# GRIPS-code/pyLBL

Measured on AMD Instinct MI355X. Metric: line×gridpoint Voigt evals/sec (whole job; per GPU: evals_per_s_per_gpu; spectra/sec: spectra_per_s), higher is better.
Workload: dtype f64; 1 GPU; BASELINE config 'target': 1 level(s) per GPU, H2O+CO2, grid 1-5000 cm-1 at 0.001 cm-1 (5000000 points), cut_off 25, remove_pedestal=False; levels_total=1, atmosphere=surface, output=gas, parallelism=levels sharded

## Files before the change

### pylbl_amd/abi.py

```python
from ctypes import CDLL, POINTER, Structure, byref, c_char_p, c_double, c_int32, c_int64, \
                   c_void_p
import os
from pathlib import Path

import numpy as np

from .errors import EngineError

LIBRARY_PATH = Path(__file__).resolve().parent / "liblbl_amd.so"

LBL_OK = 0
TABLE_OPEN_FAILED, TABLE_NO_ALIAS, TABLE_NO_TIPS, TABLE_NOT_RECTANGULAR, TABLE_NO_ISOTOPOLOGUES, \
    TABLE_NO_TRANSITIONS = 10, 11, 12, 13, 14, 15
RANGE_REFERENCE, RANGE_SKIP = 0, 1
PREP_DEVICE, PREP_HOST = 0, 1
OUT_DEVICE, ASYNC, SCALE_DENSITY, ACCUMULATE, FARFIELD, DEFER_FINISH = 1, 2, 4, 8, 16, 32
RANGE_POLICIES = {"reference": RANGE_REFERENCE, "skip": RANGE_SKIP}
PATH_OPTICAL_DEPTH, PATH_TRANSMITTANCE, PATH_CUMULATIVE, PATH_FROM_LAST, PATH_CONTINUE = \
    0x100, 0x200, 0x400, 0x800, 0x1000
PATH_RADIANCE, PATH_BRIGHTNESS = 0x2000, 0x4000
PATH_FLUX_UP = 0x8000
PATH_JACOBIAN_DEPTH, PATH_JACOBIAN_LOG_DEPTH, PATH_JACOBIAN_TEMPERATURE, \
    PATH_JACOBIAN_BOUNDARY_T, PATH_JACOBIAN_BOUNDARY_E = \
    0x10000, 0x20000, 0x40000, 0x80000, 0x100000
# ... 116 lines not shown
    "lbl_path_thermal_two_stream_source": _BLOCK + [_i32] + _RUN + [_ptr, _ptr, _f64, _ptr, _ptr,
                                                                    _ptr, _i32] + [_ptr]*10 +
                                          [_i32],
}
KDIST_PROTOTYPES = {
    "lbl_band_distribution_weighted": [_ptr, _ptr, _i64, _i64, _i32, _ptr, _i32, _ptr, _i32,
                                       _ptr, _ptr, _ptr, _ptr, _i64, _ptr, _ptr, _ptr, _i32,
                                       _ptr, _ptr, _ptr, _ptr, _ptr, _i32, _ptr, _i32],
}
SCATTERER_PROTOTYPES = {
    "lbl_path_two_stream_spectral": _BLOCK + _RUN + [_ptr, _i32, _i32, _ptr, _ptr] + [_ptr]*5 +
                                    [_i32] + [_ptr]*18 + [_i32],
    "lbl_path_thermal_two_stream_spectral": _BLOCK + [_i32] + _RUN + [_ptr, _ptr, _i32, _ptr, _ptr,
                                                                      _f64, _ptr, _ptr, _ptr,
                                                                      _i32] + [_ptr]*10 + [_i32],
}
THERMAL_RADIANCE_PROTOTYPES = {
    "lbl_path_thermal_radiance": _BLOCK + [_i32] + _RUN + [_ptr, _f64] + [_ptr]*6 + [_i32] +
                                 [_ptr]*4 + [_i32],
}
SOLAR_RADIANCE_PROTOTYPES = {
    "lbl_path_solar_radiance": _BLOCK + _RUN + [_ptr]*11 + [_i32] + [_ptr]*3 + [_i32],
}
SCATTERER_RADIANCE_PROTOTYPES = {
    "lbl_path_thermal_radiance_spectral": _BLOCK + [_i32] + _RUN + [_ptr, _i32, _ptr, _ptr, _f64] +
                                          [_ptr]*6 + [_i32] + [_ptr]*4 + [_i32],
    "lbl_path_solar_radiance_spectral": _BLOCK + _RUN + [_ptr, _i32, _i32, _ptr, _ptr] +
                                        [_ptr]*10 + [_i32] + [_ptr]*3 + [_i32],
}
THERMAL_RADIANCE_SOURCE_PROTOTYPES = {
    "lbl_path_thermal_radiance_source": _BLOCK + [_i32] + _RUN + [_ptr, _ptr, _f64] + [_ptr]*6 +
                                        [_i32] + [_ptr]*4 + [_i32],
}

_library = None


def _preload_hip_runtime():
    import importlib.util
    import os
    import sys
    from ctypes import RTLD_GLOBAL
    if "torch" in sys.modules:
        return
    try:
        spec = importlib.util.find_spec("torch")
    except (ImportError, ValueError):
        spec = None
    if spec is None or not spec.submodule_search_locations:
        return
    for location in spec.submodule_search_locations:
        candidate = os.path.join(location, "lib", "libamdhip64.so")
        if os.path.exists(candidate):
            try:
                CDLL(candidate, mode=RTLD_GLOBAL)
            except OSError:
                pass
            return


def library():
    global _library
    if _library is not None:
        return _library
    path = LIBRARY_PATH
    if os.environ.get("PYLBL_AMD_LIBRARY"):
        path = Path(os.environ["PYLBL_AMD_LIBRARY"]).resolve()
        if not path.exists():
            raise EngineError(f"$PYLBL_AMD_LIBRARY names {path}, which does not exist.")
    elif not LIBRARY_PATH.exists():
        try:
            from . import build
            build.build()
        except Exception as error:
            raise EngineError(
                f"{LIBRARY_PATH} is missing and could not be built ({error}); build it with "
                "`python -m pylbl_amd.build` (there is no CPU fallback).")
    _preload_hip_runtime()
    lib = CDLL(str(path))
    for name, arguments in list(PROTOTYPES.items()) + list(TWO_STREAM_PROTOTYPES.items()) + \
            list(THERMAL_PROTOTYPES.items()) + list(THERMAL_SOURCE_PROTOTYPES.items()) + \
            list(KDIST_PROTOTYPES.items()) + list(SCATTERER_PROTOTYPES.items()) + \
            list(THERMAL_RADIANCE_PROTOTYPES.items()) + \
            list(SOLAR_RADIANCE_PROTOTYPES.items()) + \
            list(SCATTERER_RADIANCE_PROTOTYPES.items()) + \
            list(THERMAL_RADIANCE_SOURCE_PROTOTYPES.items()):
        function = getattr(lib, name)
        function.argtypes = arguments
        function.restype = RESULT_TYPES.get(name, c_int32)
    _library = lib
    return lib


def read_line_table(path, name):
    from ctypes import create_string_buffer
    lib = library()
    table = c_void_p()
    status = lib.lbl_table_read(os.fsencode(str(path)), str(name).encode(), byref(table))
    if status != LBL_OK:
        return status, lib.lbl_last_error(None).decode(), None
    try:
        n_lines, molecule_id = c_int64(), c_int32()
        rows, num_iso, num_t = c_int32(), c_int32(), c_int32()
        formula = create_string_buffer(256)
        lib.lbl_table_shape(table, byref(n_lines), byref(molecule_id), byref(rows), byref(num_iso),
                            byref(num_t), formula, 256)
        columns = np.empty((7, n_lines.value))
        local_iso_id = np.empty(n_lines.value, dtype=np.int32)
        isoid = np.empty(rows.value, dtype=np.int64)
        mass = np.empty(rows.value)
        tips_temperature = np.empty(num_t.value)
        tips_data = np.empty((num_iso.value, num_t.value))
        lib.lbl_table_copy(table, columns.ctypes.data, local_iso_id.ctypes.data, isoid.ctypes.data,
                           mass.ctypes.data, tips_temperature.ctypes.data, tips_data.ctypes.data)
    finally:
        lib.lbl_table_free(table)
    return LBL_OK, "", {"formula": formula.value.decode(), "molecule_id": molecule_id.value,
                        "columns": columns, "local_iso_id": local_iso_id, "isoid": isoid,
                        "mass": mass, "tips_temperature": tips_temperature,
# ... 2 lines not shown
```

### pylbl_amd/csrc/accumulate.h

```cpp
#pragma once

#include <hip/hip_runtime.h>

#include "line_prep.h"
#include "voigt_profile.h"

namespace lbl {

struct Tiling
{
    int aligned;
    int per_cell;
    int length;
    int n_tiles;
};

__host__ __device__ inline void tile_bounds(const Tiling & t, int tile, int n_per_v, int n,
                                            long long & i0, long long & i1)
{
    if (t.aligned)
    {
        const int cell = tile/t.per_cell;
        const int sub = tile - cell*t.per_cell;
        i0 = (long long)cell*n_per_v + (long long)sub*t.length;
// ... 19 lines not shown
{
    const double v_lo = (double)v0 + (double)i0*dv;
    const double v_hi = (double)v0 + (double)i1*dv;
    return 0.5*(v_lo + v_hi);
}

#ifndef LBL_WING_GROUP
#define LBL_WING_GROUP 8
#endif
#ifndef LBL_FAR_TERMS
#define LBL_FAR_TERMS 21
#define LBL_FAR_RATIO 4.
#endif
constexpr int kFarTerms = LBL_FAR_TERMS;
constexpr double kFarRatio = LBL_FAR_RATIO;

struct alignas(16) WorkItem
{
    int tile;
    int part, parts;
    int slot;
};

struct AccumulateArgs
{
    const LineWing * wing;
    const LineCore * core;
    const TileSchedule * schedule;
    const LevelScalars * levels;
    const WorkItem * items;
    const double * far_series;
    const int * wing_bounds;
    int wing_batches;
    double * partial;
    long long partial_slots;
    double * k;
    long long level_stride;
    long long n_lines;
    Tiling tiling;
    int n_tiles;
    int n;
    int v0, n_per_v;
    double dv;
    double v0_real;
    int scale_density;
    int accumulate;
    int inner_everywhere;
#ifdef LBL_ABLATE
    int ablate;
#endif
};

#ifdef LBL_ABLATE
#define LBL_ABLATED(a, bits) (((a).ablate & (bits)) != 0)
#else
#define LBL_ABLATED(a, bits) false
#endif

}

#include "accumulate_lines.h"

namespace lbl {

__device__ __forceinline__ void share_of(int j0, int j1, int part, int parts, float inverse,
                                         int unit_shift, int & begin, int & end)
{
    const int units = (j1 - j0) >> unit_shift;
    const float scale = (float)units;
    const int cut0 = min((int)(scale*((float)part*inverse)), units);
    const int cut1 = min((int)(scale*((float)(part + 1)*inverse)), units);
    begin = j0 + (cut0 << unit_shift);
    end = (part + 1 == parts) ? j1 : j0 + (cut1 << unit_shift);
}

template <int P>
__device__ __forceinline__ void accumulate_tile(const AccumulateArgs & a)
{
    __shared__ double partial[4][P][64];
    const int wave = __builtin_amdgcn_readfirstlane(threadIdx.x >> 6);
    const int lane = threadIdx.x & 63;
    const int level = blockIdx.y;
    const WorkItem item = a.items[blockIdx.x];
    const int tile = item.tile;
    long long first_point, last_point;
    tile_bounds(a.tiling, tile, a.n_per_v, a.n, first_point, last_point);
    const int i0 = (int)first_point, i1 = (int)last_point;
    const TileSchedule sc = a.schedule[(long long)level*a.n_tiles + tile];
    const LineWing * __restrict__ wing = a.wing + (long long)level*a.n_lines;
    const LineCore * __restrict__ core = a.core + (long long)level*a.n_lines;

    double v[P], acc[P];
    double * slab = &partial[wave][0][0];
    __shared__ InnerStage inner_stage[4];
    const double first_index = (double)(i0 + lane);
#pragma unroll
    for (int p = 0; p < P; ++p)
    {
        const double step = (first_index + (double)(p*64))*a.dv;
        v[p] = a.v0_real + step;
        acc[p] = 0.;
    }

    const int piece = item.part*4 + wave, pieces = item.parts*4;
    GeneralList g;
    int fa0, fa1, fb0, fb1, e;
    const bool clipped_in_groups = !a.inner_everywhere && !LBL_ABLATED(a, 64);
    const float inverse = 1.f/(float)pieces;
    share_of(sc.lo, sc.a1, piece, pieces, inverse, clipped_in_groups ? 3 : 0, g.begin[0], e);
    g.count[0] = e - g.begin[0];
    share_of(sc.c1, sc.c2, piece, pieces, inverse, 0, g.begin[1], e);
    g.count[1] = e - g.begin[1];
    share_of(sc.a2, sc.hi, piece, pieces, inverse, clipped_in_groups ? 3 : 0, g.begin[2], e);
    g.count[2] = e - g.begin[2];
    share_of(sc.f1, sc.c1, piece, pieces, inverse, 2, fa0, fa1);
    share_of(sc.c2, sc.f2, piece, pieces, inverse, 2, fb0, fb1);
    g.begin[3] = fa0 + ((fa1 - fa0) & ~3);
    g.count[3] = (fa1 - fa0) & 3;
    g.begin[4] = fb0 + ((fb1 - fb0) & ~3);
    g.count[4] = (fb1 - fb0) & 3;
    if (LBL_ABLATED(a, 4)) { g.count[0] = 0; g.count[2] = 0; }
    if (LBL_ABLATED(a, 8)) { g.count[3] = 0; g.count[4] = 0; }
    if (LBL_ABLATED(a, 16)) { g.count[1] = 0; }
    if (!LBL_ABLATED(a, 2))
    {
        int batches = 1;
        if (P == 4)
        {
            const int * __restrict__ wb = a.wing_bounds + level*kWingBounds;
            const int bound[kWingBounds] = {wb[0], wb[1], wb[2], wb[3]};
            batches = __builtin_amdgcn_readfirstlane(min(wing_batches(bound), a.wing_batches));
        }
        fast_ranges<P>(wing, fa0, fa1, fb0, fb1, batches, v, acc);
    }
    bool slab_in_use = false;
    if (!LBL_ABLATED(a, 1))
    {
        GeneralList walk = g;
        if (clipped_in_groups)
        {
            clipped_ranges<P>(wing, core, g.begin[0], g.count[0], g.begin[2], g.count[2], i0, i1,
                              lane, v, acc);
            walk.count[0] = walk.count[2] = 0;
        }
        general_ranges<P>(wing, core, walk, i0, i1, lane, v, acc);
        if (!LBL_ABLATED(a, 32) && a.levels[level].inner_possible != 0.)
        {
            GeneralList inner = g;
            if (!a.inner_everywhere)
            {
                inner.count[0] = inner.count[2] = inner.count[3] = inner.count[4] = 0;
            }
            slab_in_use = inner_ranges(wing, core, inner, inner_stage[wave], i0, i1, a.v0,
                                       a.n_per_v, a.dv, lane, slab, P);
        }
    }

#pragma unroll
    for (int p = 0; p < P; ++p)
    {
        partial[wave][p][lane] = slab_in_use ? partial[wave][p][lane] + acc[p] : acc[p];
    }
    __syncthreads();

// ... 127 lines not shown
```

### pylbl_amd/csrc/accumulate_lines.h

```cpp
#pragma once

namespace lbl {

template <int P>
__device__ __forceinline__ void fast_ranges(const LineWing * __restrict__ wing,
                                            int a0, int a1, int b0, int b1, int batches,
                                            const double (&v)[P], double (&acc)[P])
{
    const int qa = (a1 - a0) >> 2;
    const int quads = qa + ((b1 - b0) >> 2);
    int q = 0;
#if LBL_WING_GROUP == 8
    auto eight = [&](int at, WingTerm (&l)[8]) {
        const int ja = at < qa ? a0 + 4*at : b0 + 4*(at - qa);
        const int jb = (at + 1) < qa ? a0 + 4*(at + 1) : b0 + 4*(at + 1 - qa);
#pragma unroll
        for (int i = 0; i < 4; ++i)
        {
            const LineWing wa = wing[ja + i], wb = wing[jb + i];
            l[i] = WingTerm{wa.centre, wa.g2, wa.bl};
            l[4 + i] = WingTerm{wb.centre, wb.g2, wb.bl};
        }
    };
    if (P == 4 && batches > 1)
// ... 23 lines not shown
                    wing_eight(v[p], l, n, t);
                    num[p] = __builtin_fma(n, den[p], num[p]*t);
                    den[p] = den[p]*t;
                }
            }
#pragma unroll
            for (int p = 0; p < P; ++p)
            {
                acc[p] = __builtin_fma(num[p], rcp_newton(den[p]), acc[p]);
            }
        }
        q = 2*eights;
    }
    for (; q + 2 <= quads; q += 2)
    {
        WingTerm l[8];
        eight(q, l);
#pragma unroll
        for (int p = 0; p < P; ++p)
        {
            acc[p] = lorentz_eight(v[p], l, acc[p]);
        }
    }
#endif
    for (; q < quads; ++q)
    {
        const int j = q < qa ? a0 + 4*q : b0 + 4*(q - qa);
        const LineWing l1 = wing[j], l2 = wing[j + 1], l3 = wing[j + 2], l4 = wing[j + 3];
#pragma unroll
        for (int p = 0; p < P; ++p)
        {
            acc[p] = lorentz_four(v[p], l1.centre, l1.g2, l1.bl, l2.centre, l2.g2, l2.bl,
                                  l3.centre, l3.g2, l3.bl, l4.centre, l4.g2, l4.bl, acc[p]);
        }
    }
}

__device__ __forceinline__ unsigned row_bits(int lo, int hi, int rows)
{
    lo = max(lo, 0);
    hi = min(hi, rows - 1);
    return lo > hi ? 0u : ((2u << hi) - 1u) & ~((1u << lo) - 1u);
}

__device__ __forceinline__ unsigned rows_meeting(int a, int b, int i0, int rows)
{
    return b < a ? 0u : row_bits((a - i0) >> 6, (b - i0) >> 6, rows);
}

__device__ __forceinline__ unsigned rows_inside(int a, int b, int i0, int rows)
{
    return b < a ? 0u : row_bits((a - i0 + 63) >> 6, (b - 63 - i0) >> 6, rows);
}

struct RegionOne
{
    double A, B, A2;
};

__device__ __forceinline__ RegionOne region_one_of(const LineCore * __restrict__ c)
{
    return RegionOne{c->A, c->B, c->A2};
}

__device__ __forceinline__ void far_quotient(const LineWing & l, double d, double & num,
                                             double & den)
// ... 455 lines not shown
```

### pylbl_amd/csrc/compute_stages.inc

```
namespace {

struct CallShape
{
    Molecule * m = nullptr;
    GridSpec g;
    long long n_long = 0;
    long long stride = 0;
    RangeRule rule;
    Tiling tiling;
    int farfield = 0;
    int points = 0;
};

int shape_of(lbl_engine * engine, const ComputeRequest & rq, CallShape & s)
{
    s.m = find_molecule(engine, rq.molecule);
    if (s.m == nullptr) return fail(engine, LBL_BAD_ARGUMENT, "unknown molecule handle.");
    if (rq.n_levels < 1 || rq.temperature == nullptr || rq.pressure == nullptr ||
        rq.vmr == nullptr)
    {
        return fail(engine, LBL_BAD_ARGUMENT, "need at least one level with T, P and x.");
    }
    if (rq.n_per_v < 1 || rq.vn <= rq.v0 || rq.cut_off < 0)
    {
// ... 144 lines not shown
                                (t.out_device ? 0 : s.n_long*8) +
                                (rq.remove_pedestal ? pedestal_bytes_per_level(n_lines, rq.vn - rq.v0, rq.cut_off) : 0);
    const long long chunk = std::max(1ll, engine->workspace_bytes/std::max(per_level, 1ll));
    return std::min<long long>(std::min<long long>(chunk, rq.n_levels), 65535);
}

struct LinesCall
{
    lbl_engine * engine;
    const ComputeRequest & rq;
    const CallShape & shape;
    const CallTraits & traits;
    Lane & lane;
    hipStream_t stream;
    const Molecule::Plan & plan;
    bool streamed;
    int pieces;
    bool with_pedestal;
    long long out_bytes;
    long long chunk;
};

void reserve_for_call(const LinesCall & c)
{
    const ComputeRequest & rq = c.rq;
    const CallShape & s = c.shape;
    const CallTraits & t = c.traits;
    Lane & lane = c.lane;
    const long long n_lines = s.m->n_lines, n_tiles = s.tiling.n_tiles, chunk = c.chunk;
    lane.level_feed.refill((size_t)chunk);
    lane.levels.reserve((size_t)chunk);
    lane.wing.reserve((size_t)(chunk*std::max(n_lines, 1ll)));
    lane.core.reserve((size_t)(chunk*std::max(n_lines, 1ll)));
    lane.schedule.reserve((size_t)(chunk*n_tiles));
    if (t.want_k && !t.out_device) lane.staging.reserve((size_t)(chunk*s.n_long));
    if (c.with_pedestal && t.out_device && t.add_into_block)
    {
        lane.raw.reserve((size_t)(chunk*s.n_long));
    }
    if (t.want_k && s.farfield)
    {
        lane.far_series.reserve((size_t)(chunk*n_tiles*kFarTerms));
    }
    if (t.want_k)
    {
        lane.partial.reserve((size_t)std::max(1ll, chunk*c.plan.partial_slots*64*s.points));
    }
    lane.wing_bounds.reserve((size_t)(chunk*kWingBounds));
    if (rq.evals != nullptr)
    {
        lane.evals.reserve(1);
        HIP_TRY(hipMemsetAsync(lane.evals.data, 0, sizeof(unsigned long long), c.stream));
    }
    if (rq.derived != nullptr) lane.derived.reserve((size_t)(std::max(n_lines, 1ll)*8));
}

void launch_far_series(lbl_engine * engine, Lane & lane, const CallShape & s, int count,
                       hipStream_t stream)
{
    const GridSpec & g = s.g;
    const int n_tiles = s.tiling.n_tiles;
    const int n_groups = (n_tiles + kFarGroup - 1)/kFarGroup;
    const long long n_lines = s.m->n_lines;
    engine->timed(kTimeSchedule, stream, [&] {
        dim3 far_grid((unsigned)(((n_groups + 7)/8)*8), (unsigned)count);
        hipLaunchKernelGGL(farfield_series_kernel, far_grid, dim3(256), 0, stream, lane.wing.data,
// ... 39 lines not shown
    for (int l = 0; l < count; ++l)
    {
        std::string why;
        LevelScalars & lv = lane.level_feed.block[l];
        if (!fill_level(*c.shape.m, rq.temperature[base + l], rq.pressure[base + l],
                        rq.vmr[base + l], lv, why))
        {
            return fail(c.engine, LBL_OUT_OF_RANGE,
                        "level " + std::to_string(base + l) + ": " + why);
        }
        bound_inner_regions(*c.shape.m, c.shape.rule, lv);
    }
    if (!levels_inline(c.engine, count))
    {
        lane.level_feed.upload(lane.levels.data, (size_t)count, c.stream);
    }
    return LBL_OK;
}

int inner_points_everywhere(const LevelScalars * levels, int count, const ComputeRequest & rq,
                            const CallShape & s)
{
    double reach = 0.;
    for (int l = 0; l < count; ++l)
    {
        const LevelScalars & lv = levels[l];
        const double kk = lv.core_reach;
        reach = std::max(reach, kk < 0.5 ? kk*(rq.vn + 1.)/(1. - kk) + 2.*lv.shift_max : 1.e9);
    }
    const double tile_width = (double)s.tiling.length*s.g.dv;
    return (rq.cut_off - 1. <= reach + tile_width + 1.) ? 1 : 0;
}

struct HostPrep
{
    std::vector<LineWing> wing;
    std::vector<LineCore> core;
    std::vector<double> derived;
    std::vector<int> wing_bounds;
};

void prepare_on_host(lbl_engine * engine, Lane & lane, const ComputeRequest & rq,
                     const CallShape & s, int count, hipStream_t stream, HostPrep & hp)
{
    const Molecule & m = *s.m;
    const long long n_lines = m.n_lines;
    if (n_lines > 0)
    {
        hp.wing.resize((size_t)(count*n_lines));
        hp.core.resize((size_t)(count*n_lines));
        if (rq.derived != nullptr) hp.derived.assign((size_t)(n_lines*8), 0.);
        hp.wing_bounds.assign((size_t)(count*kWingBounds), kWingBoundsFill);
        unsigned long long total = 0;
        for (int l = 0; l < count; ++l)
        {
            for (long long j = 0; j < n_lines; ++j)
            {
                const bool ok = m.iso_slot[j] >= 0 &&
                                line_accepted(s.rule, m.column[0][j], m.order[j]);
                double * d = (rq.derived != nullptr && l == 0) ? hp.derived.data() + j*8
                                                               : nullptr;
                LineWing & w = hp.wing[(size_t)(l*n_lines + j)];
                const int status = prepare_line(
                    lane.level_feed.block[l], s.g, m.column[0][j], m.column[1][j], m.column[2][j],
                    m.column[3][j], m.column[4][j], m.column[5][j], m.column[6][j],
                    std::max(m.iso_slot[j], 0), ok, w, hp.core[(size_t)(l*n_lines + j)], d);
                if (status == 1 && w.last >= w.first) total += w.last - w.first + 1;
                int bound[kWingBounds];
                wing_line_bounds(s.g, m.column[0][j], status, w,
                                 hp.core[(size_t)(l*n_lines + j)], bound);
                for (int b = 0; b < kWingBounds; ++b)
                {
                    int & least = hp.wing_bounds[(size_t)(l*kWingBounds + b)];
                    least = std::min(least, bound[b]);
                }
            }
        }
        engine->timed(kTimePrepare, stream, [&] {
            HIP_TRY(hipMemcpyAsync(lane.wing.data, hp.wing.data(),
                                   hp.wing.size()*sizeof(LineWing), hipMemcpyHostToDevice,
                                   stream));
            HIP_TRY(hipMemcpyAsync(lane.core.data, hp.core.data(),
                                   hp.core.size()*sizeof(LineCore), hipMemcpyHostToDevice,
                                   stream));
            HIP_TRY(hipMemcpyAsync(lane.wing_bounds.data, hp.wing_bounds.data(),
                                   hp.wing_bounds.size()*sizeof(int), hipMemcpyHostToDevice,
                                   stream));
        });
        HIP_TRY(hipStreamSynchronize(stream));
        if (rq.evals != nullptr) *rq.evals += (int64_t)total;
    }
    if (rq.k != nullptr)
    {
        engine->timed(kTimeSchedule, stream, [&] {
            dim3 grid((unsigned)((8ll*s.tiling.n_tiles + 255)/256), (unsigned)count);
            hipLaunchKernelGGL(schedule_kernel, grid, dim3(256), 0, stream, m.view(),
                               lane.levels.data, s.g, s.tiling, s.farfield, lane.schedule.data);
            HIP_TRY(hipGetLastError());
        });
    }
}

void launch_prologue(const LinesCall & c, int count, HostPrep & hp)
{
    lbl_engine * engine = c.engine;
    const ComputeRequest & rq = c.rq;
    const CallShape & s = c.shape;
    Lane & lane = c.lane;
    hipStream_t stream = c.stream;
    if (engine->prep == LBL_PREP_HOST)
    {
        prepare_on_host(engine, lane, rq, s, count, stream, hp);
        return;
    }
    const bool inline_levels = levels_inline(engine, count);
    InlineLevels packed;
    if (inline_levels)
    {
        std::memcpy(packed.level, lane.level_feed.block, count*sizeof(LevelScalars));
    }
    const int prepare_blocks = (int)((s.m->n_lines + 255)/256);
    const int schedule_blocks = c.traits.want_k ? (int)((8ll*s.tiling.n_tiles + 255)/256) : 0;
    HIP_TRY(hipMemsetAsync(lane.wing_bounds.data, 0x7f, (size_t)count*kWingBounds*sizeof(int),
                           stream));
    engine->timed(kTimePrepare, stream, [&] {
        dim3 grid((unsigned)std::max(prepare_blocks + schedule_blocks, 1), (unsigned)count);
        hipLaunchKernelGGL(prologue_kernel, grid, dim3(256), 0, stream, s.m->view(),
                           lane.levels.data, packed, inline_levels ? 1 : 0, s.g, s.rule, s.tiling,
                           s.farfield, prepare_blocks, lane.wing.data, lane.core.data,
                           lane.schedule.data,
                           rq.derived != nullptr ? lane.derived.data : nullptr,
                           rq.evals != nullptr ? lane.evals.data : nullptr,
                           lane.wing_bounds.data);
        HIP_TRY(hipGetLastError());
    });
}

Lane::Pass pass_of(const LinesCall & c, long long base, int count)
{
    const CallTraits & t = c.traits;
    Lane::Pass p;
    p.base = base;
    p.count = count;
    p.target = t.out_device ? c.rq.k + base*c.shape.stride : c.lane.staging.data;
    p.target_stride = t.out_device ? c.shape.stride : c.shape.n_long;
    p.sums = p.target;
    p.sums_stride = p.target_stride;
    if (c.with_pedestal && t.out_device && t.add_into_block)
    {
        p.sums = c.lane.raw.data;
        p.sums_stride = c.shape.n_long;
    }
    p.ped_stream = c.engine->overlap_pedestal ? c.lane.side : c.stream;
    p.finish_stream = c.with_pedestal ? p.ped_stream : c.stream;
    return p;
}

void start_pedestal_search(const LinesCall & c, const Lane::Pass & p)
{
    lbl_engine * engine = c.engine;
    Lane & lane = c.lane;
    if (engine->overlap_pedestal)
    {
        lane.prepared.record(c.stream);
        HIP_TRY(hipStreamWaitEvent(lane.side, lane.prepared, 0));
    }
    engine->timed(kTimePedestal, p.ped_stream, [&] {
        pedestal_find_runs(lane.pedestal, p.ped_stream, c.shape.m->view(), lane.wing.data,
                           c.shape.g, p.count, c.rq.vn - c.rq.v0, engine->scan_chain != 0,
                           engine->poison_workspace != 0);
    }, 0);
    if (engine->overlap_pedestal)
    {
        lane.runs_found.record(lane.side);
    }
}

AccumulateArgs accumulate_args(const LinesCall & c, const Lane::Pass & p)
{
    const ComputeRequest & rq = c.rq;
    const CallShape & s = c.shape;
    const GridSpec & g = s.g;
    const Lane & lane = c.lane;
    const bool add_into = c.traits.out_device && c.traits.add_into_block;
    AccumulateArgs args;
    args.wing = lane.wing.data;
    args.core = lane.core.data;
    args.schedule = lane.schedule.data;
    args.levels = lane.levels.data;
    args.items = c.plan.items.data;
    args.far_series = s.farfield ? lane.far_series.data : nullptr;
    args.wing_bounds = lane.wing_bounds.data;
    args.wing_batches = c.engine->wing_batches;
    args.partial = lane.partial.data;
    args.partial_slots = c.plan.partial_slots;
    args.level_stride = p.sums_stride;
    args.k = p.sums;
    args.n_lines = s.m->n_lines;
    args.tiling = s.tiling;
    args.n_tiles = s.tiling.n_tiles;
    args.n = g.n;
    args.v0 = g.v0;
    args.n_per_v = g.n_per_v;
    args.dv = g.dv;
    args.v0_real = (double)g.v0;
    args.scale_density = (!c.with_pedestal && (rq.flags & LBL_SCALE_DENSITY)) ? 1 : 0;
    args.accumulate = (!c.with_pedestal && add_into) ? 1 : 0;
    args.inner_everywhere = inner_points_everywhere(lane.level_feed.block, p.count, rq, s);
#ifdef LBL_ABLATE
    args.ablate = c.engine->ablate;
#endif
    return args;
}

void launch_piece(const LinesCall & c, const Lane::Pass & p, const AccumulateArgs & args,
                  int piece)
{
    const Molecule::Plan & plan = c.plan;
    hipStream_t stream = c.stream;
    const int points = c.shape.points, count = p.count;
    const int item0 = plan.item_begin[piece], item1 = plan.item_begin[piece + 1];
    const int split0 = plan.split_begin[piece], split1 = plan.split_begin[piece + 1];
    c.engine->timed(kTimeAccumulate, stream, [&] {
        if (item1 > item0)
        {
            AccumulateArgs mine = args;
// ... 165 lines not shown
```

### pylbl_amd/csrc/engine.hip

```cpp
#include <hip/hip_runtime.h>

#include <algorithm>
#include <cmath>
#include <cstdio>
#include <cstring>
#include <functional>
#include <limits>
#include <memory>
#include <mutex>
#include <numeric>
#include <string>
#include <vector>

#include "../../include/lbl_amd.h"
#include "../../include/lbl_amd_twostream.h"
#include "../../include/lbl_amd_thermal.h"
#include "../../include/lbl_amd_thermal_source.h"
#include "../../include/lbl_amd_kdist.h"
#include "../../include/lbl_amd_scatterer.h"
#include "../../include/lbl_amd_thermal_radiance.h"
#include "../../include/lbl_amd_solar_radiance.h"
#include "../../include/lbl_amd_scatterer_radiance.h"
#include "../../include/lbl_amd_thermal_radiance_source.h"
#include "accumulate.h"
#include "band_sort.h"
#include "band_sort_pairs.h"
#include "continuum.h"
#include "xsec.h"
#include "farfield.h"
#include "flux.h"
#include "instrument.h"
#include "jacobian.h"
#include "line_prep.h"
#include "path.h"
#include "pedestal.h"
#include "radiance.h"
#include "solar.h"
#include "surface.h"
#include "tile_schedule.h"
#include "twostream.h"
#include "twostream_thermal.h"
#include "thermal_radiance.h"
#include "thermal_radiance_source.h"
#include "solar_radiance.h"

#include "engine_core.h"
#include "lanes_plans.inc"
#include "compute_stages.inc"
#include "compute_call.inc"

#include "delivery.inc"
#include "slot_entry.inc"

extern "C" {

const char * lbl_version(void)
{
    return "pylbl_amd 0.1 (gfx950)";
}

int lbl_wing_batches(const int32_t * bounds)
{
    if (bounds == nullptr) return 1;
    const int bound[kWingBounds] = {bounds[0], bounds[1], bounds[2], bounds[3]};
    return wing_batches(bound);
}

int lbl_engine_create(int device, lbl_engine ** engine)
{
    if (engine == nullptr) return fail(nullptr, LBL_BAD_ARGUMENT, "engine is NULL.");
    *engine = nullptr;
    int count = 0;
    if (hipGetDeviceCount(&count) != hipSuccess || count <= 0)
    {
        return fail(nullptr, LBL_NO_DEVICE,
                    "no HIP device visible: this engine has no CPU fallback.");
    }
    if (device < 0 || device >= count)
    {
        return fail(nullptr, LBL_NO_DEVICE, "device index out of range.");
    }
    try
    {
        HIP_TRY(hipSetDevice(device));
        std::unique_ptr<lbl_engine> e(new lbl_engine());
        e->device = device;
        for (int i = 0; i < kAllLanes; ++i) e->lanes[i].create(i == kSlotLane);
        e->stream = e->lanes[0].main;
        e->copy_stream.create();
        calibrate_delivery_lanes(e.get());
        e->copies_handed_over.create();
        e->taken_over.create();
        *engine = e.release();
    }
    catch (const HipFailure & f)
    {
        return fail(nullptr, LBL_NO_DEVICE, f.message);
    }
// ... 397 lines not shown
```

### pylbl_amd/csrc/engine_core.h

```cpp
#pragma once

#include "hip_owners.h"

namespace {

using namespace lbl;

thread_local std::string g_create_error;
thread_local std::string g_thread_error;
thread_local const void * g_thread_error_engine = nullptr;

struct Molecule
{
    long long n_lines = 0;
    std::vector<double> nu_row;
    bool ascending = true;
    std::vector<int> order;
    std::vector<double> column[7];
    std::vector<int> iso_slot;
    double mass[kMassSlots];
    unsigned used_slots = 0;
    struct BadRow { int row; double nu; int local_iso_id; };
    std::vector<BadRow> bad_rows;
    double max_abs_delta = 0.;
// ... 61 lines not shown
    struct Pass
    {
        long long base = 0;
        int count = 0;
        double * target = nullptr;
        long long target_stride = 0;
        double * sums = nullptr;
        long long sums_stride = 0;
        hipStream_t ped_stream = nullptr;
        hipStream_t finish_stream = nullptr;
    };
    struct Finish
    {
        bool pending = false;
        Pass pass;
        GridSpec g;
        int pieces = 1, flags = 0;
        long long point_begin[9] = {};
        bool streamed = false, order_writers = false, add_into = false;
        char * host = nullptr;
        long long host_pitch = 0, columns = 0;
        double * k = nullptr;
        const double * block = nullptr;
        long long out_bytes = 0;
    } finish;
    struct Write { const char * begin = nullptr; const char * end = nullptr; Event done; };
    static constexpr int kWrites = 4;
    Write writes[kWrites];
    int next_write = 0;
    bool writes_wrapped = false;
    bool used = false;
    DeviceBuffer<LineWing> wing;
    DeviceBuffer<LineCore> core;
    DeviceBuffer<TileSchedule> schedule;
    DeviceBuffer<LevelScalars> levels;
    DeviceBuffer<double> staging;
    DeviceBuffer<double> raw;
    DeviceBuffer<double> partial;
    DeviceBuffer<double> far_series;
    DeviceBuffer<double> derived;
    DeviceBuffer<unsigned long long> evals;
    DeviceBuffer<int> wing_bounds;
    PedestalWorkspace pedestal;
    PinnedFeed<LevelScalars> level_feed;

    void create(bool urgent = false)
    {
        main.create(urgent);
        side.create(true);
        for (Event * e : {&prepared, &pedestal_done, &runs_found, &queued, &handed_over,
                          &level_feed.copied})
        {
            e->create();
        }
        for (auto & e : piece_done) e.create();
        for (auto & e : piece_summed) e.create();
        for (auto & w : writes) w.done.create();
    }
    void drain()
    {
        main.drain();
        side.drain();
    }
    ~Lane() { drain(); }
    void note_write(const void * begin, long long bytes, hipStream_t stream)
    {
// ... 394 lines not shown
```

### pylbl_amd/csrc/line_prep.h

```cpp
#pragma once

#include <hip/hip_runtime.h>
#include <math.h>
#include <stdint.h>

namespace lbl {

constexpr int kMassSlots = 32;
constexpr double kPi = 3.14159265358979323846;

struct LevelScalars
{
    double temperature;
    double p_atm;
    double p_partial;
    double tfact;
    double t_minus_ref;
    double t_times_ref;
    double shift_max;
    double core_reach;
    double density;
    double inner_possible;
    double doppler[kMassSlots];
    double q_ratio[kMassSlots];
// ... 108 lines not shown
    {
        const double v = fmax(fabs((double)g.v0), fabs((double)g.vn));
        bound[kWingTHighNeg] = -wing_exponent_high(v*v + 1.);
    }
}

__host__ __device__ inline int wing_batches(const int (&bound)[kWingBounds])
{
    const long long t_lo = bound[kWingTLow], t_hi = -(long long)bound[kWingTHighNeg];
    long long b_lo = bound[kWingBLow], b_hi = -(long long)bound[kWingBHighNeg];
    if (t_lo == kWingBoundsFill || -t_hi == kWingBoundsFill)
    {
        return 1;
    }
    if (b_lo == kWingBoundsFill)
    {
        b_lo = b_hi = 0;
    }
    if (t_lo < -2000 || t_hi > 2000 || b_lo < -2000 || b_hi > 2000)
    {
        return 1;
    }
    for (int k = kWingBatchesMax; k > 1; k >>= 1)
    {
        const long long n = 8*k;
        const long long lowest = (t_lo < 0 ? n*t_lo : (n - 1)*t_lo) + (b_lo < 0 ? b_lo : 0);
        const long long highest = (t_hi > 0 ? n*t_hi : (n - 1)*t_hi) + (b_hi > 0 ? b_hi : 0) + 6;
        if (lowest >= -1000 && highest <= 1000 && n*t_lo >= -1000 && n*t_hi <= 1000)
        {
            return k;
        }
    }
    return 1;
}

__host__ __device__ inline int prepare_line(const LevelScalars & lv, const GridSpec & g,
                                            double nu, double sw, double gamma_air,
                                            double gamma_self, double n_air, double elower,
                                            double delta_air, int iso_slot, bool accepted,
                                            LineWing & w, LineCore & c, double * derived)
{
    const double vlight = 2.99792458e8;
    const double c2 = 1.4387752;
    const double rsqrpi = 1./sqrt(kPi);
    const double sqrln2 = sqrt(log(2.));
    mark_empty(w, c);
    if (derived != nullptr)
    {
        for (int i = 0; i < 8; ++i) derived[i] = 0.;
        derived[6] = -1.;
    }
    if (!accepted)
    {
        return -1;
    }
    const double centre = nu + lv.p_atm*delta_air;
    const double gamma = (gamma_air*(lv.p_atm - lv.p_partial) + gamma_self*lv.p_partial)*
                         pow(lv.tfact, n_air);
    const double alpha = (nu/vlight)*lv.doppler[iso_slot];
    const double sb = exp(elower*c2*lv.t_minus_ref/lv.t_times_ref);
    const double gg = exp((-c2*nu)/lv.temperature);
    const double gref = exp((-c2*nu)/296.);
    const double se = (1. - gg)/(1. - gref);
    const double strength = sw*sb*se*lv.q_ratio[iso_slot]*0.01*0.01;

    const double fl = floor(centre);
// ... 72 lines not shown
```

### pylbl_amd/csrc/tile_schedule.h

```cpp
#pragma once

#include <hip/hip_runtime.h>

#include "accumulate.h"
#include "line_prep.h"

namespace lbl {

struct LineTableView
{
    const double * nu;
    const double * sw;
    const double * gamma_air;
    const double * gamma_self;
    const double * n_air;
    const double * elower;
    const double * delta_air;
    const int * iso_slot;
    const int * row;
    const int * sorted_of_row;
    long long n_lines;
    const int * cell_first;
    double cell_base, cell_scale;
    int cell_entries;
// ... 121 lines not shown
        s.f1 = min(max(value[6], s.a1), s.c1);
        s.f2 = min(max(value[7], s.c2), s.a2);
    }
    *out = s;
}

__global__ __launch_bounds__(256) void schedule_kernel(const LineTableView table,
                                                       const LevelScalars * __restrict__ levels,
                                                       const GridSpec g, const Tiling tiling,
                                                       const int farfield,
                                                       TileSchedule * __restrict__ schedule)
{
    const int thread = blockIdx.x*blockDim.x + threadIdx.x;
    const int tile = thread >> 3;
    const int level = blockIdx.y;
    const bool active = tile < tiling.n_tiles;
    schedule_tile(table, levels[level], g, tiling, farfield, tile, thread & 7, active,
                  schedule + (long long)level*tiling.n_tiles + (active ? tile : 0));
}

constexpr int kInlineLevels = 4;
struct InlineLevels
{
    LevelScalars level[kInlineLevels];
};

__device__ __forceinline__ void prepare_block(const LineTableView & t, const LevelScalars & lv,
                                              const GridSpec & g, const RangeRule & rule,
                                              int block, int level,
                                              LineWing * __restrict__ wing,
                                              LineCore * __restrict__ core,
                                              double * __restrict__ derived,
                                              unsigned long long * __restrict__ evals,
                                              int * __restrict__ wing_bounds)
{
    const long long j = (long long)block*blockDim.x + threadIdx.x;
    unsigned long long count = 0;
    int bound[kWingBounds] = {kWingBoundsFill, kWingBoundsFill, kWingBoundsFill, kWingBoundsFill};
    if (j < t.n_lines)
    {
        LineWing w;
        LineCore c;
        const double nu = t.nu[j];
        const int slot = t.iso_slot[j];
        const bool ok = slot >= 0 && line_accepted(rule, nu, t.row[j]);
        double * d = derived != nullptr ? derived + ((long long)level*t.n_lines + j)*8 : nullptr;
        const int status = prepare_line(lv, g, nu, t.sw[j], t.gamma_air[j],
                                        t.gamma_self[j], t.n_air[j], t.elower[j],
                                        t.delta_air[j], max(slot, 0), ok, w, c, d);
        wing[(long long)level*t.n_lines + j] = w;
        core[(long long)level*t.n_lines + j] = c;
        if (status == 1 && w.last >= w.first)
        {
            count = (unsigned long long)(w.last - w.first + 1);
        }
        wing_line_bounds(g, nu, status, w, c, bound);
    }
    {
        __shared__ int block_bound[4][kWingBounds];
#pragma unroll
        for (int b = 0; b < kWingBounds; ++b)
        {
            for (int offset = 32; offset > 0; offset >>= 1)
            {
                bound[b] = min(bound[b], __shfl_down(bound[b], offset, 64));
            }
        }
        const int wave = threadIdx.x >> 6;
        if ((threadIdx.x & 63) == 0)
        {
#pragma unroll
            for (int b = 0; b < kWingBounds; ++b) block_bound[wave][b] = bound[b];
        }
        __syncthreads();
        if (threadIdx.x < kWingBounds)
        {
            const int b = threadIdx.x;
            const int least = min(min(block_bound[0][b], block_bound[1][b]),
                                  min(block_bound[2][b], block_bound[3][b]));
            if (least != kWingBoundsFill)
            {
                atomicMin(wing_bounds + (long long)level*kWingBounds + b, least);
            }
        }
    }
    if (evals != nullptr)
    {
        for (int offset = 32; offset > 0; offset >>= 1)
        {
            count += __shfl_down(count, offset, 64);
        }
        if ((threadIdx.x & 63) == 0 && count != 0)
        {
            atomicAdd(evals, count);
        }
    }
}

__global__ __launch_bounds__(256) void prologue_kernel(const LineTableView t,
                                                       LevelScalars * __restrict__ levels,
                                                       const InlineLevels inline_levels,
                                                       const int use_inline,
                                                       const GridSpec g, const RangeRule rule,
                                                       const Tiling tiling, const int farfield,
                                                       const int prepare_blocks,
                                                       LineWing * __restrict__ wing,
                                                       LineCore * __restrict__ core,
                                                       TileSchedule * __restrict__ schedule,
                                                       double * __restrict__ derived,
                                                       unsigned long long * __restrict__ evals,
                                                       int * __restrict__ wing_bounds)
{
    const int level = blockIdx.y;
    const LevelScalars & lv = use_inline ? inline_levels.level[level] : levels[level];
    if (use_inline && blockIdx.x == 0)
    {
        const double * from = reinterpret_cast<const double *>(&inline_levels.level[level]);
        double * to = reinterpret_cast<double *>(levels + level);
        for (int i = threadIdx.x; i < (int)(sizeof(LevelScalars)/8); i += blockDim.x) to[i] = from[i];
    }
    if ((int)blockIdx.x < prepare_blocks)
    {
        prepare_block(t, lv, g, rule, blockIdx.x, level, wing, core, derived, evals,
                      wing_bounds);
        return;
    }
    const int thread = (blockIdx.x - prepare_blocks)*blockDim.x + threadIdx.x;
    const int tile = thread >> 3;
    const bool active = tile < tiling.n_tiles;
    schedule_tile(t, lv, g, tiling, farfield, tile, thread & 7, active,
                  schedule + (long long)level*tiling.n_tiles + (active ? tile : 0));
}

}
```

### pylbl_amd/csrc/voigt_profile.h

```cpp
#pragma once

#include <hip/hip_runtime.h>

namespace lbl {

__device__ __forceinline__ double rcp_newton(double t)
{
    double r = __builtin_amdgcn_rcp(t);
    double e = __builtin_fma(-t, r, 1.0);
    return __builtin_fma(r, e, r);
}

__device__ __forceinline__ double lorentz_one(double v, double centre, double g2, double bl,
                                              double sum)
{
    const double d = v - centre;
    return __builtin_fma(bl, rcp_newton(__builtin_fma(d, d, g2)), sum);
}

__device__ __forceinline__ double lorentz_four(double v,
                                               double c1, double g1, double b1,
                                               double c2, double g2, double b2,
                                               double c3, double g3, double b3,
                                               double c4, double g4, double b4, double sum)
{
    const double d1 = v - c1, d2 = v - c2, d3 = v - c3, d4 = v - c4;
    const double t1 = __builtin_fma(d1, d1, g1);
    const double t2 = __builtin_fma(d2, d2, g2);
    const double t3 = __builtin_fma(d3, d3, g3);
    const double t4 = __builtin_fma(d4, d4, g4);
    const double n12 = __builtin_fma(b1, t2, b2*t1);
    const double n34 = __builtin_fma(b3, t4, b4*t3);
    const double t12 = t1*t2, t34 = t3*t4;
    const double num = __builtin_fma(n12, t34, n34*t12);
    return __builtin_fma(num, rcp_newton(t12*t34), sum);
}

struct WingTerm
{
    double centre, g2, bl;
};

__device__ __forceinline__ void wing_pair(double v, const WingTerm & p, const WingTerm & q,
                                          double & num, double & den)
{
    const double d1 = v - p.centre, d2 = v - q.centre;
    const double t1 = __builtin_fma(d1, d1, p.g2);
    const double t2 = __builtin_fma(d2, d2, q.g2);
    num = __builtin_fma(p.bl, t2, q.bl*t1);
    den = t1*t2;
}

__device__ __forceinline__ void wing_eight(double v, const WingTerm (&l)[8],
                                           double & num, double & den)
{
    double n12, t12, n34, t34, n56, t56, n78, t78;
    wing_pair(v, l[0], l[1], n12, t12);
    wing_pair(v, l[2], l[3], n34, t34);
    wing_pair(v, l[4], l[5], n56, t56);
    wing_pair(v, l[6], l[7], n78, t78);
    const double na = __builtin_fma(n12, t34, n34*t12), ta = t12*t34;
    const double nb = __builtin_fma(n56, t78, n78*t56), tb = t56*t78;
    num = __builtin_fma(na, tb, nb*ta);
    den = ta*tb;
}

__device__ __forceinline__ double lorentz_eight(double v, const WingTerm (&l)[8], double sum)
{
    double num, den;
    wing_eight(v, l, num, den);
    return __builtin_fma(num, rcp_newton(den), sum);
}


template <int N>
__device__ __forceinline__ double horner(const double (&c)[N], double t)
{
    double value = c[N - 1];
#pragma unroll
    for (int k = N - 2; k >= 0; --k)
    {
        value = c[k] + t*value;
    }
    return value;
}

struct InnerLimits
{
    double two, three, four;
};

__device__ __forceinline__ InnerLimits inner_limits(double y)
{
    InnerLimits lim;
    lim.two = (y <= 0.000001) ? 1.e300 : 6.8 - y;
    lim.three = 2.4*y;
    lim.four = 18.1*y + 1.65;
// ... 202 lines not shown
```

Baseline: 6433 billion evals/s.

## Evaluate far-wing Lorentz lines in pre-scaled groups of eight

Wing lines are packed into groups of eight during line preparation. Each line is rescaled by a shared geometric-mean strength beta and a shared centre offset m, so the group's rational sum needs only one fma chain per line instead of separate strength multiplies and pairwise combines. The accumulation kernel (P==4 tiles past a threshold) consumes these groups through a new scaled_ranges path. Groups whose strengths span too wide an exponent range, or that fail normality checks, fall back to the plain eight-line Lorentz evaluation. The cost is extra preparation work, an extra 208-byte record per group to store and read, and a ballot-driven fallback pass over the groups.

```diff
diff --git a/include/lbl_amd_wing.h b/include/lbl_amd_wing.h
--- /dev/null
+++ b/include/lbl_amd_wing.h
@@ -0,0 +1,17 @@
+#ifndef LBL_AMD_WING_H_
+#define LBL_AMD_WING_H_
+
+#include "lbl_amd.h"
+
+#ifdef __cplusplus
+extern "C" {
+#endif
+
+int lbl_wing_group(const double *centre, const double *g2, const double *bl, int32_t lines,
+                   double *record);
+
+#ifdef __cplusplus
+}
+#endif
+
+#endif
diff --git a/pylbl_amd/abi.py b/pylbl_amd/abi.py
--- a/pylbl_amd/abi.py
+++ b/pylbl_amd/abi.py
@@ -172,6 +172,9 @@
     "lbl_path_thermal_radiance_source": _BLOCK + [_i32] + _RUN + [_ptr, _ptr, _f64] + [_ptr]*6 +
                                         [_i32] + [_ptr]*4 + [_i32],
 }
+WING_PROTOTYPES = {
+    "lbl_wing_group": [_ptr, _ptr, _ptr, _i32, _ptr],
+}
 
 _library = None
 
@@ -224,7 +227,7 @@
             list(THERMAL_RADIANCE_PROTOTYPES.items()) + \
             list(SOLAR_RADIANCE_PROTOTYPES.items()) + \
             list(SCATTERER_RADIANCE_PROTOTYPES.items()) + \
-            list(THERMAL_RADIANCE_SOURCE_PROTOTYPES.items()):
+            list(THERMAL_RADIANCE_SOURCE_PROTOTYPES.items()) + list(WING_PROTOTYPES.items()):
         function = getattr(lib, name)
         function.argtypes = arguments
         function.restype = RESULT_TYPES.get(name, c_int32)
diff --git a/pylbl_amd/csrc/accumulate.h b/pylbl_amd/csrc/accumulate.h
--- a/pylbl_amd/csrc/accumulate.h
+++ b/pylbl_amd/csrc/accumulate.h
@@ -75,6 +75,9 @@
     const double * far_series;
     const int * wing_bounds;
     int wing_batches;
+    const WingGroup * groups;
+    int group_base;
+    int scaled_from;
     double * partial;
     long long partial_slots;
     double * k;
@@ -117,6 +120,24 @@
     end = (part + 1 == parts) ? j1 : j0 + (cut1 << unit_shift);
 }
 
+__device__ __forceinline__ void aligned_share_of(int j0, int j1, int part, int parts,
+                                                 float inverse, int base, int & s0,
+                                                 int & s1, int & r0, int & r1)
+{
+    const int first = base + ((max(j0, base) - base + 7) & ~7);
+    const int last = j1 > base ? base + ((j1 - base) & ~7) : first;
+    if (first >= last)
+    {
+        s0 = s1 = first;
+        r0 = j0;
+        r1 = part == 0 ? j1 : j0;
+        return;
+    }
+    share_of(first, last, part, parts, inverse, 3, s0, s1);
+    r0 = part + 1 == parts ? last : j0;
+    r1 = part + 1 == parts ? j1 : (part == 0 ? first : j0);
+}
+
 template <int P>
 __device__ __forceinline__ void accumulate_tile(const AccumulateArgs & a)
 {
@@ -156,8 +177,17 @@
     g.count[1] = e - g.begin[1];
     share_of(sc.a2, sc.hi, piece, pieces, inverse, clipped_in_groups ? 3 : 0, g.begin[2], e);
     g.count[2] = e - g.begin[2];
-    share_of(sc.f1, sc.c1, piece, pieces, inverse, 2, fa0, fa1);
-    share_of(sc.c2, sc.f2, piece, pieces, inverse, 2, fb0, fb1);
+    int sa0 = 0, sa1 = 0, sb0 = 0, sb1 = 0;
+    if (P == 4 && i0 >= a.scaled_from)
+    {
+        aligned_share_of(sc.f1, sc.c1, piece, pieces, inverse, a.group_base, sa0, sa1, fa0, fa1);
+        aligned_share_of(sc.c2, sc.f2, piece, pieces, inverse, a.group_base, sb0, sb1, fb0, fb1);
+    }
+    else
+    {
+        share_of(sc.f1, sc.c1, piece, pieces, inverse, 2, fa0, fa1);
+        share_of(sc.c2, sc.f2, piece, pieces, inverse, 2, fb0, fb1);
+    }
     g.begin[3] = fa0 + ((fa1 - fa0) & ~3);
     g.count[3] = (fa1 - fa0) & 3;
     g.begin[4] = fb0 + ((fb1 - fb0) & ~3);
@@ -173,6 +203,12 @@
             const int * __restrict__ wb = a.wing_bounds + level*kWingBounds;
             const int bound[kWingBounds] = {wb[0], wb[1], wb[2], wb[3]};
             batches = __builtin_amdgcn_readfirstlane(min(wing_batches(bound), a.wing_batches));
+        }
+        if constexpr (P == 4)
+        {
+            const WingGroup * __restrict__ groups =
+                a.groups + (long long)level*((a.n_lines + 7) >> 3);
+            scaled_ranges(wing, groups, a.group_base, sa0, sa1, sb0, sb1, batches, lane, v, acc);
         }
         fast_ranges<P>(wing, fa0, fa1, fb0, fb1, batches, v, acc);
     }
diff --git a/pylbl_amd/csrc/accumulate_lines.h b/pylbl_amd/csrc/accumulate_lines.h
--- a/pylbl_amd/csrc/accumulate_lines.h
+++ b/pylbl_amd/csrc/accumulate_lines.h
@@ -79,6 +79,90 @@
         {
             acc[p] = lorentz_four(v[p], l1.centre, l1.g2, l1.bl, l2.centre, l2.g2, l2.bl,
                                   l3.centre, l3.g2, l3.bl, l4.centre, l4.g2, l4.bl, acc[p]);
+        }
+    }
+}
+
+template <bool First>
+__device__ __forceinline__ void scaled_batch(const WingGroup * __restrict__ g,
+                                             const double (&v)[4], double (&num)[4],
+                                             double (&den)[4])
+{
+    const double beta = g->beta, m = g->m;
+    double s[8], gs[8], nas[8];
+#pragma unroll
+    for (int i = 0; i < 8; ++i)
+    {
+        nas[i] = g->nas[i];
+        s[i] = g->s[i];
+        gs[i] = g->gs[i];
+    }
+#pragma unroll
+    for (int p = 0; p < 4; ++p)
+    {
+        double n, t;
+        scaled_eight(v[p] - m, s, nas, gs, n, t);
+        n = beta*n;
+        if (First)
+        {
+            num[p] = n;
+            den[p] = t;
+        }
+        else
+        {
+            num[p] = __builtin_fma(n, den[p], num[p]*t);
+            den[p] = den[p]*t;
+        }
+    }
+}
+
+__device__ __forceinline__ void scaled_ranges(const LineWing * __restrict__ wing,
+                                              const WingGroup * __restrict__ groups, int group_base,
+                                              int a0, int a1, int b0, int b1, int batches,
+                                              int lane, const double (&v)[4], double (&acc)[4])
+{
+    a0 = __builtin_amdgcn_readfirstlane(a0);
+    b0 = __builtin_amdgcn_readfirstlane(b0);
+    const int ea = __builtin_amdgcn_readfirstlane((a1 - a0) >> 3);
+    const int eights = ea + __builtin_amdgcn_readfirstlane((b1 - b0) >> 3);
+    auto line_of = [&](int at) { return at < ea ? a0 + 8*at : b0 + 8*(at - ea); };
+    auto group_of = [&](int at) { return groups + ((line_of(at) - group_base) >> 3); };
+    for (int o = 0; o < eights; )
+    {
+        const int stop = min(o + batches, eights);
+        double num[4], den[4];
+        scaled_batch<true>(group_of(o), v, num, den);
+        for (++o; o < stop; ++o)
+        {
+            scaled_batch<false>(group_of(o), v, num, den);
+        }
+#pragma unroll
+        for (int p = 0; p < 4; ++p)
+        {
+            acc[p] = __builtin_fma(num[p], rcp_newton(den[p]), acc[p]);
+        }
+    }
+    for (int base = 0; base < eights; base += 64)
+    {
+        const int at = min(base + lane, eights - 1);
+        const bool plain = base + lane < eights && !(group_of(at)->beta != 0.);
+        unsigned long long left = __ballot(plain);
+        while (left != 0)
+        {
+            const int j = line_of(base + __builtin_ctzll(left));
+            WingTerm l[8];
+#pragma unroll
+            for (int i = 0; i < 8; ++i)
+            {
+                const LineWing w = wing[j + i];
+                l[i] = WingTerm{w.centre, w.g2, w.bl};
+            }
+#pragma unroll
+            for (int p = 0; p < 4; ++p)
+            {
+                acc[p] = lorentz_eight(v[p], l, acc[p]);
+            }
+            left &= left - 1;
         }
     }
 }
diff --git a/pylbl_amd/csrc/compute_stages.inc b/pylbl_amd/csrc/compute_stages.inc
--- a/pylbl_amd/csrc/compute_stages.inc
+++ b/pylbl_amd/csrc/compute_stages.inc
@@ -200,6 +200,7 @@
     lane.levels.reserve((size_t)chunk);
     lane.wing.reserve((size_t)(chunk*std::max(n_lines, 1ll)));
     lane.core.reserve((size_t)(chunk*std::max(n_lines, 1ll)));
+    lane.groups.reserve((size_t)(chunk*std::max((n_lines + 7) >> 3, 1ll)));
     lane.schedule.reserve((size_t)(chunk*n_tiles));
     if (t.want_k && !t.out_device) lane.staging.reserve((size_t)(chunk*s.n_long));
     if (c.with_pedestal && t.out_device && t.add_into_block)
@@ -305,10 +306,18 @@
     return (rq.cut_off - 1. <= reach + tile_width + 1.) ? 1 : 0;
 }
 
+long long wing_group_base(const CallShape & s)
+{
+    const std::vector<double> & nu = s.m->column[0];
+    return (long long)(std::lower_bound(nu.begin(), nu.begin() + s.m->n_lines, s.rule.nu_min) -
+                       nu.begin());
+}
+
 struct HostPrep
 {
     std::vector<LineWing> wing;
     std::vector<LineCore> core;
+    std::vector<WingGroup> groups;
     std::vector<double> derived;
     std::vector<int> wing_bounds;
 };
@@ -349,6 +358,29 @@
                 }
             }
         }
+        const long long base = wing_group_base(s);
+        const long long n_groups = s.points == 4 ? (n_lines - base + 7) >> 3 : 0;
+        const long long group_stride = (n_lines + 7) >> 3;
+        hp.groups.assign((size_t)(count*group_stride), WingGroup());
+        for (int l = 0; l < count; ++l)
+        {
+            for (long long group = 0; group < n_groups; ++group)
+            {
+                double centre[8], g2[8], bl[8];
+                const long long first = base + 8*group;
+                const int lines = (int)std::min(8ll, n_lines - first);
+                for (int i = 0; i < 8; ++i)
+                {
+                    const bool real = i < lines;
+                    const LineWing * w = real ? &hp.wing[(size_t)(l*n_lines + first + i)]
+                                              : nullptr;
+                    centre[i] = real ? w->centre : 0.;
+                    g2[i] = real ? w->g2 : 1.;
+                    bl[i] = real ? w->bl : 0.;
+                }
+                wing_group_of(centre, g2, bl, lines, hp.groups[(size_t)(l*group_stride + group)]);
+            }
+        }
         engine->timed(kTimePrepare, stream, [&] {
             HIP_TRY(hipMemcpyAsync(lane.wing.data, hp.wing.data(),
                                    hp.wing.size()*sizeof(LineWing), hipMemcpyHostToDevice,
@@ -356,6 +388,9 @@
             HIP_TRY(hipMemcpyAsync(lane.core.data, hp.core.data(),
                                    hp.core.size()*sizeof(LineCore), hipMemcpyHostToDevice,
                                    stream));
+            HIP_TRY(hipMemcpyAsync(lane.groups.data, hp.groups.data(),
+                                   hp.groups.size()*sizeof(WingGroup), hipMemcpyHostToDevice,
+                                   stream));
             HIP_TRY(hipMemcpyAsync(lane.wing_bounds.data, hp.wing_bounds.data(),
                                    hp.wing_bounds.size()*sizeof(int), hipMemcpyHostToDevice,
                                    stream));
@@ -392,7 +427,7 @@
     {
         std::memcpy(packed.level, lane.level_feed.block, count*sizeof(LevelScalars));
     }
-    const int prepare_blocks = (int)((s.m->n_lines + 255)/256);
+    const int prepare_blocks = (int)((s.m->n_lines + 8 + 255)/256);
     const int schedule_blocks = c.traits.want_k ? (int)((8ll*s.tiling.n_tiles + 255)/256) : 0;
     HIP_TRY(hipMemsetAsync(lane.wing_bounds.data, 0x7f, (size_t)count*kWingBounds*sizeof(int),
                            stream));
@@ -404,7 +439,8 @@
                            lane.schedule.data,
                            rq.derived != nullptr ? lane.derived.data : nullptr,
                            rq.evals != nullptr ? lane.evals.data : nullptr,
-                           lane.wing_bounds.data);
+                           lane.wing_bounds.data,
+                           s.points == 4 ? lane.groups.data : nullptr, (int)wing_group_base(s));
         HIP_TRY(hipGetLastError());
     });
 }
@@ -465,6 +501,13 @@
     args.far_series = s.farfield ? lane.far_series.data : nullptr;
     args.wing_bounds = lane.wing_bounds.data;
     args.wing_batches = c.engine->wing_batches;
+    args.groups = lane.groups.data;
+    args.group_base = (int)wing_group_base(s);
+    {
+        const long long gate = std::max(64ll, 2ll*((long long)g.cut_off + 2));
+        const long long from = std::max(0ll, gate - (long long)g.v0)*(long long)g.n_per_v;
+        args.scaled_from = (int)std::min(from, 0x7fffffffll);
+    }
     args.partial = lane.partial.data;
     args.partial_slots = c.plan.partial_slots;
     args.level_stride = p.sums_stride;
diff --git a/pylbl_amd/csrc/engine.hip b/pylbl_amd/csrc/engine.hip
--- a/pylbl_amd/csrc/engine.hip
+++ b/pylbl_amd/csrc/engine.hip
@@ -22,6 +22,7 @@
 #include "../../include/lbl_amd_solar_radiance.h"
 #include "../../include/lbl_amd_scatterer_radiance.h"
 #include "../../include/lbl_amd_thermal_radiance_source.h"
+#include "../../include/lbl_amd_wing.h"
 #include "accumulate.h"
 #include "band_sort.h"
 #include "band_sort_pairs.h"
@@ -64,6 +65,31 @@
     if (bounds == nullptr) return 1;
     const int bound[kWingBounds] = {bounds[0], bounds[1], bounds[2], bounds[3]};
     return wing_batches(bound);
+}
+
+int lbl_wing_group(const double * centre, const double * g2, const double * bl, int32_t lines,
+                   double * record)
+{
+    if (centre == nullptr || g2 == nullptr || bl == nullptr || record == nullptr) return -1;
+    double c[8], g[8], b[8];
+    for (int i = 0; i < 8; ++i)
+    {
+        const bool real = i < lines;
+        c[i] = real ? centre[i] : 0.;
+        g[i] = real ? g2[i] : 1.;
+        b[i] = real ? bl[i] : 0.;
+    }
+    WingGroup group;
+    wing_group_of(c, g, b, std::min(std::max((int)lines, 0), 8), group);
+    for (int i = 0; i < 8; ++i)
+    {
+        record[3*i] = group.s[i];
+        record[3*i + 1] = group.nas[i];
+        record[3*i + 2] = group.gs[i];
+    }
+    record[24] = group.beta;
+    record[25] = group.m;
+    return group.beta != 0. ? 1 : 0;
 }
 
 int lbl_engine_create(int device, lbl_engine ** engine)
diff --git a/pylbl_amd/csrc/engine_core.h b/pylbl_amd/csrc/engine_core.h
--- a/pylbl_amd/csrc/engine_core.h
+++ b/pylbl_amd/csrc/engine_core.h
@@ -117,6 +117,7 @@
     bool used = false;
     DeviceBuffer<LineWing> wing;
     DeviceBuffer<LineCore> core;
+    DeviceBuffer<WingGroup> groups;
     DeviceBuffer<TileSchedule> schedule;
     DeviceBuffer<LevelScalars> levels;
     DeviceBuffer<double> staging;
diff --git a/pylbl_amd/csrc/line_prep.h b/pylbl_amd/csrc/line_prep.h
--- a/pylbl_amd/csrc/line_prep.h
+++ b/pylbl_amd/csrc/line_prep.h
@@ -164,6 +164,114 @@
         }
     }
     return 1;
+}
+
+struct WingScaled
+{
+    double s, nas, gs;
+};
+
+struct alignas(16) WingGroup
+{
+    double s[8];
+    double gs[8];
+    double nas[8];
+    double beta;
+    double m;
+};
+static_assert(sizeof(WingGroup) == 208, "WingGroup is read by wide loads: 26 doubles");
+
+__host__ __device__ inline void wing_group_set(WingGroup & g, int i, const WingScaled & l)
+{
+    g.s[i] = l.s;
+    g.nas[i] = l.nas;
+    g.gs[i] = l.gs;
+}
+
+constexpr WingScaled kWingPlainLine = {0., 0., 1.};
+constexpr double kWingGroupReach = 1.5;
+constexpr int kWingGroupSpread = 128;
+
+__host__ __device__ inline bool wing_is_normal(double x)
+{
+    const double a = fabs(x);
+    return a >= 2.2250738585072014e-308 && a <= 1.7976931348623157e308;
+}
+
+__host__ __device__ inline double wing_group_beta(const double (&bl)[8])
+{
+    double mantissa = 1.;
+    int exponent = 0;
+    for (int i = 0; i < 8; ++i)
+    {
+        int e;
+        mantissa *= frexp(bl[i], &e);
+        exponent += e;
+    }
+    const int q = exponent >> 3, r = exponent & 7;
+    return ldexp(sqrt(sqrt(sqrt(ldexp(mantissa, r)))), q);
+}
+
+__host__ __device__ inline bool wing_group_header(double first_centre, const double (&bl)[8],
+                                                  int lines, double & beta, double & m)
+{
+    beta = 0.;
+    m = 0.;
+    if (lines < 8 || !(fabs(first_centre) < 4.e15))
+    {
+        return false;
+    }
+    int low = 4096, high = -4096;
+    for (int i = 0; i < 8; ++i)
+    {
+        if (!(bl[i] > 0.) || !wing_is_normal(bl[i]))
+        {
+            return false;
+        }
+        const int e = ilogb(bl[i]);
+        low = e < low ? e : low;
+        high = e > high ? e : high;
+    }
+    if (high - low > kWingGroupSpread)
+    {
+        return false;
+    }
+    beta = wing_group_beta(bl);
+    m = rint(first_centre);
+    return wing_is_normal(beta);
+}
+
+__host__ __device__ inline bool wing_group_line(double centre, double g2, double bl, double beta,
+                                                double m, WingScaled & out)
+{
+    const double a = centre - m;
+    const double s = sqrt(beta/bl);
+    out.s = s;
+    out.nas = -(a*s);
+    out.gs = g2*(s*s);
+    return fabs(a) <= kWingGroupReach && wing_is_normal(s) && wing_is_normal(out.gs) &&
+           fabs(out.nas) <= 1.7976931348623157e308;
+}
+
+__host__ __device__ inline void wing_group_of(const double (&centre)[8], const double (&g2)[8],
+                                              const double (&bl)[8], int lines, WingGroup & out)
+{
+    double beta, m;
+    bool scaled = wing_group_header(centre[0], bl, lines, beta, m);
+    for (int i = 0; i < 8; ++i)
+    {
+        WingScaled l;
+        scaled = wing_group_line(centre[i], g2[i], bl[i], beta, m, l) && scaled;
+        wing_group_set(out, i, l);
+    }
+    out.beta = beta;
+    out.m = m;
+    if (!scaled)
+    {
+        for (int i = 0; i < 8; ++i) wing_group_set(out, i, kWingPlainLine);
+        out.beta = 0.;
+        out.m = 0.;
+    }
 }
 
 __host__ __device__ inline int prepare_line(const LevelScalars & lv, const GridSpec & g,
diff --git a/pylbl_amd/csrc/tile_schedule.h b/pylbl_amd/csrc/tile_schedule.h
--- a/pylbl_amd/csrc/tile_schedule.h
+++ b/pylbl_amd/csrc/tile_schedule.h
@@ -177,14 +177,16 @@
                                               LineCore * __restrict__ core,
                                               double * __restrict__ derived,
                                               unsigned long long * __restrict__ evals,
-                                              int * __restrict__ wing_bounds)
-{
-    const long long j = (long long)block*blockDim.x + threadIdx.x;
+                                              int * __restrict__ wing_bounds,
+                                              WingGroup * __restrict__ groups, int group_base)
+{
+    const long long j = (long long)block*blockDim.x + threadIdx.x + ((group_base & 7) - 8);
     unsigned long long count = 0;
     int bound[kWingBounds] = {kWingBoundsFill, kWingBoundsFill, kWingBoundsFill, kWingBoundsFill};
-    if (j < t.n_lines)
-    {
-        LineWing w;
+    LineWing w;
+    w.centre = 0.; w.g2 = 1.; w.bl = 0.;
+    if (j >= 0 && j < t.n_lines)
+    {
         LineCore c;
         const double nu = t.nu[j];
         const int slot = t.iso_slot[j];
@@ -200,6 +202,34 @@
             count = (unsigned long long)(w.last - w.first + 1);
         }
         wing_line_bounds(g, nu, status, w, c, bound);
+    }
+    if (groups != nullptr)
+    {
+        const int lane = threadIdx.x & 63, leader = lane & ~7;
+        double bl[8];
+#pragma unroll
+        for (int i = 0; i < 8; ++i) bl[i] = __shfl(w.bl, leader + i, 64);
+        const double first_centre = __shfl(w.centre, leader, 64);
+        const long long first_line = j - (lane - leader);
+        const int lines = first_line < group_base ? 0
+                        : (int)min(8ll, max(0ll, t.n_lines - first_line));
+        double beta, m;
+        WingScaled mine;
+        bool scaled = wing_group_header(first_centre, bl, lines, beta, m);
+        scaled = wing_group_line(w.centre, w.g2, w.bl, beta, m, mine) && scaled;
+        const unsigned long long agree = __ballot(scaled);
+        scaled = ((agree >> leader) & 0xffull) == 0xffull;
+        if (j >= group_base && j < t.n_lines)
+        {
+            WingGroup * __restrict__ out = groups + (long long)level*((t.n_lines + 7) >> 3) +
+                                           ((j - group_base) >> 3);
+            wing_group_set(*out, lane - leader, scaled ? mine : kWingPlainLine);
+            if (lane == leader)
+            {
+                out->beta = scaled ? beta : 0.;
+                out->m = scaled ? m : 0.;
+            }
+        }
     }
     {
         __shared__ int block_bound[4][kWingBounds];
@@ -254,7 +284,9 @@
                                                        TileSchedule * __restrict__ schedule,
                                                        double * __restrict__ derived,
                                                        unsigned long long * __restrict__ evals,
-                                                       int * __restrict__ wing_bounds)
+                                                       int * __restrict__ wing_bounds,
+                                                       WingGroup * __restrict__ groups,
+                                                       const int group_base)
 {
     const int level = blockIdx.y;
     const LevelScalars & lv = use_inline ? inline_levels.level[level] : levels[level];
@@ -267,7 +299,7 @@
     if ((int)blockIdx.x < prepare_blocks)
     {
         prepare_block(t, lv, g, rule, blockIdx.x, level, wing, core, derived, evals,
-                      wing_bounds);
+                      wing_bounds, groups, group_base);
         return;
     }
     const int thread = (blockIdx.x - prepare_blocks)*blockDim.x + threadIdx.x;
diff --git a/pylbl_amd/csrc/voigt_profile.h b/pylbl_amd/csrc/voigt_profile.h
--- a/pylbl_amd/csrc/voigt_profile.h
+++ b/pylbl_amd/csrc/voigt_profile.h
@@ -1,6 +1,8 @@
 #pragma once
 
 #include <hip/hip_runtime.h>
+
+#include "line_prep.h"
 
 namespace lbl {
 
@@ -63,6 +65,27 @@
     const double nb = __builtin_fma(n56, t78, n78*t56), tb = t56*t78;
     num = __builtin_fma(na, tb, nb*ta);
     den = ta*tb;
+}
+
+__device__ __forceinline__ void scaled_eight(double u, const double (&s)[8],
+                                             const double (&nas)[8], const double (&gs)[8],
+                                             double & num, double & den)
+{
+    const double d0 = __builtin_fma(u, s[0], nas[0]);
+    const double d1 = __builtin_fma(u, s[1], nas[1]);
+    const double t0 = __builtin_fma(d0, d0, gs[0]);
+    const double t1 = __builtin_fma(d1, d1, gs[1]);
+    double N = t0 + t1, T = t0*t1;
+#pragma unroll
+    for (int i = 2; i < 8; ++i)
+    {
+        const double d = __builtin_fma(u, s[i], nas[i]);
+        const double t = __builtin_fma(d, d, gs[i]);
+        N = __builtin_fma(N, t, T);
+        T = T*t;
+    }
+    num = N;
+    den = T;
 }
 
 __device__ __forceinline__ double lorentz_eight(double v, const WingTerm (&l)[8], double sum)
```

Result: faster. 6633 billion evals/s (median of 6 runs) (+3.1%).
